# DataCanvasIO/DeepTables

Measured on AMD Instinct MI355X. Metric: training rows/sec (fwd+bwd) DeepFM Criteo-shape batch 8192, higher is better.
Workload: dtype f32 (split-bf16: 24-bit fwd / 16-bit bwd)

## Files before the change

### deeptables_amd/csrc/deepfm.hip

```cpp
#include <stdlib.h>
#include "tile_common.h"
#include "tower_x3.h"
#include "adam_dev.h"

namespace dt {

typedef float floatx4_t __attribute__((ext_vector_type(4)));

struct DeepFmAccum {
    int64_t dW1, dW2, db1, db2, dw3, dwo, dbo, loss, dgamma, dbeta, dwlin, slin, total;
    int64_t dw3d, dcw, dcb, sumc, sumcx;
};
__host__ __device__ inline DeepFmAccum deepfm_accum_layout(int C, int CP, int F, int Nd, int L = 0) {
    DeepFmAccum a;
    int64_t o = 0;
    a.dW1 = o; o += (int64_t)C * kH1;
    a.dW2 = o; o += (int64_t)kH1 * kH2;
    a.db1 = o; o += kH1;
    a.db2 = o; o += kH2;
    a.dw3 = o; o += (L > 0 ? C : 0);
    a.dw3d = o; o += kH2;
    a.dwo = o; o += 1;
    a.dbo = o; o += 1;
    a.loss = o; o += 2;
// ... 1528 lines not shown
                    acc[t][u] = __builtin_amdgcn_mfma_f32_32x32x16_bf16(al[t], bh[u], acc[t][u], 0, 0, 0);
                }
                acc[t][u] = __builtin_amdgcn_mfma_f32_32x32x16_bf16(ah[t], bh[u], acc[t][u], 0, 0, 0);
            }
    }
    auto put = [&](float* slot) {
#pragma unroll
        for (int t = 0; t < 2; ++t)
#pragma unroll
            for (int r = 0; r < 16; ++r) {
                const int i = (r & 3) + 8 * (r >> 2) + 4 * s;
                st4(slot + (2 * i + t) * 128 + 4 * c, floatx4{acc[t][0][r], acc[t][1][r], acc[t][2][r], acc[t][3][r]});
            }
    };
    put(red + wave * 8192);
    if (soft_cnt) {
        asm volatile("s_waitcnt lgkmcnt(0)" ::: "memory");
        if (lane == 0) atomicAdd(soft_cnt, 1u);
        while (*reinterpret_cast<volatile unsigned*>(soft_cnt) < 4u) __builtin_amdgcn_s_sleep(1);
        asm volatile("" ::: "memory");
    } else {
        __syncthreads();
    }
    float* dst = wpart + ((int64_t)mac * row_blocks + rb) * 8192;
#pragma unroll
    for (int u = 0; u < 8; ++u) {
        const int e = 4 * (tid + 256 * u);
        st4(dst + e, (ld4(red + e) + ld4(red + 8192 + e)) + (ld4(red + 16384 + e) + ld4(red + 24576 + e)));
    }
}

struct GPart {
    const float* part;
    int stride, tiles;
    float* gsum;
};
__device__ __forceinline__ void reduce_gpart(const GPart& gp, float* lds, int blk, int nblk, int tid, ElectSync& sy) {
    const int ee = tid & 15, tg = tid >> 4;
    for (int e0 = 16 * blk; e0 < gp.stride; e0 += 16 * nblk) {
        float acc = 0.f;
        for (int t0 = tg; t0 < gp.tiles; t0 += 16 * 8) {
            float v[8];
#pragma unroll
            for (int u = 0; u < 8; ++u) {
                const int t = t0 + 16 * u;
                const float x = gp.part[(int64_t)min(t, gp.tiles - 1) * gp.stride + e0 + ee];
                v[u] = t < gp.tiles ? x : 0.f;
            }
            acc += ((v[0] + v[1]) + (v[2] + v[3])) + ((v[4] + v[5]) + (v[6] + v[7]));
        }
        elect_barrier<256, true>(sy);
        lds[tg * 16 + ee] = acc;
        elect_barrier<256, true>(sy);
        if (tid < 16) {
            float t = 0.f;
#pragma unroll
            for (int g = 0; g < 16; ++g) t += lds[g * 16 + tid];
            gp.gsum[e0 + tid] = t;
        }
    }
}
struct X3Lay {
    __bf16 *W1B, *W1R, *W2B, *W2R;
    int64_t w1b_lo, w1r_lo, w2b_lo, w2r_lo;
    float* cwp;
};
__device__ __forceinline__ void x3_parts(float v, __bf16 (&q)[3]) {
    float r = v;
#pragma unroll
    for (int k = 0; k < 3; ++k) {
        const __bf16 a = (__bf16)r;
        q[k] = a;
        r -= (float)a;
    }
}

__device__ __forceinline__ void bn_grads2_body(const float* __restrict__ W1, const float* __restrict__ gamma,
                                               const float* __restrict__ beta, const DeepFmDims& dm, float* accum,
                                               const DeepFmAccum& al, const float* __restrict__ wpart, int row_blocks,
                                               int Lc, const float* __restrict__ cw, const float* __restrict__ cb,
                                               const float* __restrict__ w3c, const RecSrc& rs, const Part3& pl,
                                               floatx2 (*sm)[64], float* slin_s, const DenseAdam& da, int blk, const GPart& gp,
                                               const X3Lay& lay = X3Lay{nullptr, nullptr, nullptr, nullptr, 0, 0, 0, 0, nullptr}) {
    const int lane = threadIdx.x & 63, wave = threadIdx.x >> 6;
    if (blk == 0 && Lc == 0) {
        float* sl = reinterpret_cast<float*>(slin_s);
        for (int c = threadIdx.x; c < dm.C; c += blockDim.x) sl[c] = rec_sum(rs, pl.slin + c);
        __syncthreads();
        for (int q = threadIdx.x; q < dm.F + dm.Nd; q += blockDim.x) {
            float v = 0.f;
            if (q < dm.F) {
                for (int d = 0; d < dm.D; ++d) v += sl[q * dm.D + d];
            } else {
                v = sl[dm.F * dm.D + (q - dm.F)];
            }
            accum[al.dwlin + q] = v;
            if (da.p) adam_one(da.p, da.m, da.v, al.dwlin + q, v, da.lr_t, da.b1, da.b2, da.eps);
        }
    }
    const int col = blk;
    const bool w2 = col >= dm.C;
    const int mac = w2 ? (dm.CP >> 6) : (col >> 6), row = w2 ? col - dm.C : (col & 63);
    const float* src = wpart + (int64_t)mac * row_blocks * 8192 + row * 128 + 2 * lane;
    floatx2 w = {0.f, 0.f}, d = {0.f, 0.f};
    float ga = 0.f, be = 0.f;
    typedef double doublex2 __attribute__((ext_vector_type(2)));
    doublex2 dq[kRecShards];
#pragma unroll
    for (int sh = 0; sh < kRecShards; ++sh) dq[sh] = doublex2{0.0, 0.0};
    if (wave == 0 && !w2) {
        w = *reinterpret_cast<const floatx2*>(W1 + (int64_t)col * kH1 + 2 * lane);
#pragma unroll
        for (int sh = 0; sh < kRecShards; ++sh)
            dq[sh] = *reinterpret_cast<const doublex2*>(rs.racc + (int64_t)sh * rs.stride + pl.db1 + 2 * lane);
        ga = gamma[col]; be = beta[col];
    }
    const int64_t e0 = w2 ? al.dW2 + (int64_t)(2 * lane) * kH2 + row : al.dW1 + (int64_t)col * kH1 + 2 * lane;
    const int64_t e1 = w2 ? e0 + kH2 : e0 + 1;
    float pp[2] = {0.f, 0.f}, pm[2] = {0.f, 0.f}, pv[2] = {0.f, 0.f};
    if (da.p && wave == 0) {
        pp[0] = da.p[e0]; pp[1] = da.p[e1]; pm[0] = da.m[e0]; pm[1] = da.m[e1]; pv[0] = da.v[e0]; pv[1] = da.v[e1];
    }
    float pnew[2] = {0.f, 0.f};
    auto adam2 = [&](float g0, float g1) {
        const float g[2] = {g0, g1};
        const int64_t ei[2] = {e0, e1};
#pragma unroll
        for (int k = 0; k < 2; ++k) {
            const float mi = da.b1 * pm[k] + (1.f - da.b1) * g[k];
            const float vi = da.b2 * pv[k] + (1.f - da.b2) * g[k] * g[k];
            da.m[ei[k]] = mi;
            da.v[ei[k]] = vi;
            pnew[k] = pp[k] - da.lr_t * mi / (sqrtf(vi) + da.eps);
            da.p[ei[k]] = pnew[k];
        }
    };
    floatx2 v[8];
#pragma unroll
    for (int u = 0; u < 8; ++u) {
        const int sl = wave + 4 * u;
        v[u] = floatx2{0.f, 0.f};
        if (sl < row_blocks) v[u] = *reinterpret_cast<const floatx2*>(src + (int64_t)sl * 8192);
    }
    floatx2 m = ((v[0] + v[1]) + (v[2] + v[3])) + ((v[4] + v[5]) + (v[6] + v[7]));
    for (int sl = wave + 32; sl < row_blocks; sl += 4) m += *reinterpret_cast<const floatx2*>(src + (int64_t)sl * 8192);
    sm[wave][lane] = m;
    __syncthreads();
    if (wave != 0) return;
    m = (sm[0][lane] + sm[1][lane]) + (sm[2][lane] + sm[3][lane]);
    {
        doublex2 t = dq[0];
#pragma unroll
        for (int sh = 1; sh < kRecShards; ++sh) t += dq[sh];
        d = floatx2{(float)t[0], (float)t[1]};
    }
    if (w2) {
        accum[e0] = m.x;
        accum[e1] = m.y;
        if (da.p) adam2(m.x, m.y);
        if (da.p && lay.W1B) {
            __bf16 q0[3], q1[3];
            x3_parts(pnew[0], q0);
            x3_parts(pnew[1], q1);
            const int k0 = 2 * lane, n = row;
            const int64_t ib = ((((int64_t)(k0 >> 5) * 4 + (n >> 4)) * 64) + ((k0 >> 3) & 3) * 16 + (n & 15)) * 8 + (k0 & 7);
#pragma unroll
            for (int pt = 0; pt < 3; ++pt) {
// ... 20 lines not shown
            x3_parts(pnew[0], q0);
            x3_parts(pnew[1], q1);
            const int k = col, n0 = 2 * lane;
            const int64_t kb = ((int64_t)(k >> 5) * 8) * 64 * 8 + (((k >> 3) & 3) * 16) * 8 + (k & 7);
            const int64_t i0 = kb + ((int64_t)(n0 >> 4) * 64 + (n0 & 15)) * 8, i1 = kb + ((int64_t)((n0 + 1) >> 4) * 64 + ((n0 + 1) & 15)) * 8;
#pragma unroll
            for (int pt = 0; pt < 3; ++pt) {
                lay.W1B[pt * lay.w1b_lo + i0] = q0[pt];
                lay.W1B[pt * lay.w1b_lo + i1] = q1[pt];
            }
#pragma unroll
            for (int pt = 0; pt < 2; ++pt) {
                typedef __bf16 b2 __attribute__((ext_vector_type(2)));
                *reinterpret_cast<b2*>(lay.W1R + pt * lay.w1r_lo + (int64_t)k * kH1 + n0) = b2{q0[pt], q1[pt]};
            }
        }
    }
    if (Lc) {
        const int scal = pl.cross + (Lc + 1) * dm.CP;
        const int l = lane;
        const float sa_mine = l < Lc ? rec_sum(rs, scal + 16 + l) : 0.f;
        const float sco_mine = l <= Lc ? rec_sum(rs, scal + l) : 0.f;
        const float G = l <= Lc ? gp.gsum[(int64_t)l * dm.CP + col] : 0.f;
        const float sdz = rec_sum(rs, scal + 31);
        float cl = 0.f, suf = 0.f;
        for (int j = 0; j < Lc; ++j) {
            const float saj = __shfl(sa_mine, j, 64);
            const float bj = cb[(int64_t)j * dm.C + col], wj = cw[(int64_t)j * dm.C + col];
            if (j < l) cl += bj;
            if (j > l) suf += saj * wj;
        }
        if (l <= Lc) {
            const int64_t ig = l < Lc ? al.dcw + (int64_t)l * dm.C + col : al.dw3 + col;
            const float gw = ga_b * G + be_b * sco_mine + (l < Lc ? sa_mine : sdz) * cl;
            const float gb = sdz * w3c[col] + suf;
            accum[ig] = gw;
            if (l < Lc) accum[al.dcb + (int64_t)l * dm.C + col] = gb;
            if (da.p) {
                adam_one(da.p, da.m, da.v, ig, gw, da.lr_t, da.b1, da.b2, da.eps);
                if (l < Lc) adam_one(da.p, da.m, da.v, al.dcb + (int64_t)l * dm.C + col, gb, da.lr_t, da.b1, da.b2, da.eps);
                if (lay.cwp) {
                    lay.cwp[(int64_t)(l < Lc ? l : 2 * Lc) * dm.CP + col] = da.p[ig];
                    if (l < Lc) lay.cwp[(int64_t)(Lc + l) * dm.CP + col] = da.p[al.dcb + (int64_t)l * dm.C + col];
                }
            }
        }
    }
}

__global__ __launch_bounds__(256) void k_bn_grads2(const float* __restrict__ W1, const float* __restrict__ gamma,
                                                   const float* __restrict__ beta, DeepFmDims dm, float* accum,
                                                   DeepFmAccum al, const float* __restrict__ wpart, int row_blocks,
                                                   int Lc, const float* __restrict__ cw, const float* __restrict__ cb,
                                                   const float* __restrict__ w3c, RecSrc rs, int col_blocks, GPart gp) {
    __shared__ floatx2 sm[4][64];
    __shared__ float slin_s[kMaxC];
    const DenseAdam none{nullptr, nullptr, nullptr, 0.f, 0.f, 0.f, 0.f};
    const Part3 pl = part3_layout(dm.CP, Lc, 1);
    if ((int)blockIdx.x < col_blocks)
        bn_grads2_body(W1, gamma, beta, dm, accum, al, wpart, row_blocks, Lc, cw, cb, w3c, rs, pl, sm, slin_s, none, (int)blockIdx.x, gp);
    else
        finish_record_entry(((int)blockIdx.x - col_blocks) * (int)blockDim.x + (int)threadIdx.x, rs, pl, al, dm, Lc, accum, none);
}

__global__ __launch_bounds__(256) void k_finish_records(DeepFmDims dm, float* accum, DeepFmAccum al, int Lc, RecSrc rs,
                                                        double* __restrict__ bnacc_zero, int bnacc_n) {
    const DenseAdam none{nullptr, nullptr, nullptr, 0.f, 0.f, 0.f, 0.f};
    const Part3 pl = part3_layout(dm.CP, Lc, 0);
    const int i = (int)blockIdx.x * (int)blockDim.x + (int)threadIdx.x;
    finish_record_entry(i, rs, pl, al, dm, Lc, accum, none);
    for (int j = i; j < bnacc_n; j += (int)(gridDim.x * blockDim.x)) bnacc_zero[j] = 0.0;
}

struct FinishSeg {
    SegTail seg;
    float *table, *m, *v;
    const float* values;
    int sstride, D;
};
__global__ __launch_bounds__(256) void k_finish_step(const float* __restrict__ W1, const float* __restrict__ gamma,
                                                     const float* __restrict__ beta, DeepFmDims dm, float* accum,
                                                     DeepFmAccum al, const float* __restrict__ wpart, int row_blocks,
                                                     DenseAdam da, AdamState* __restrict__ st, float lr, int col_blocks,
                                                     int small_blocks, int seg_blocks, FinishSeg fs, int Lc,
                                                     const float* __restrict__ cw, const float* __restrict__ cb,
                                                     const float* __restrict__ w3c, RecSrc rs, X3Lay lay, GPart gp,
                                                     const float* __restrict__ lr_snap) {
    __shared__ floatx2 sm[4][64];
    __shared__ float slin_s[kMaxC];
    const Part3 pl = part3_layout(dm.CP, Lc, 1);
    const int sb = (int)blockIdx.x < seg_blocks ? (int)blockIdx.x : -1;
    const int b = sb >= 0 ? col_blocks + small_blocks : (int)blockIdx.x - seg_blocks < small_blocks
                      ? col_blocks + ((int)blockIdx.x - seg_blocks) : (int)blockIdx.x - seg_blocks - small_blocks;
    int nseg0 = 0;
    if (sb >= 0 && fs.seg.nseg) nseg0 = fs.seg.nseg[(sb * (int)(blockDim.x >> 6) + (int)(threadIdx.x >> 6)) % fs.seg.regions];
    if (lr_snap) da.lr_t = *lr_snap; else if (st) da.lr_t = st->lr_t;
    if (b < col_blocks) {
        bn_grads2_body(W1, gamma, beta, dm, accum, al, wpart, row_blocks, Lc, cw, cb, w3c, rs, pl, sm, slin_s, da, b, gp, lay);
    } else if (b < col_blocks + small_blocks) {
        finish_record_entry((b - col_blocks) * (int)blockDim.x + (int)threadIdx.x, rs, pl, al, dm, Lc, accum, da);
    } else if (fs.seg.nseg) {
        adam_segments<true>(fs.seg, seg_blocks, nseg0, fs.table, fs.m, fs.v, fs.values, fs.D, da.lr_t, da.b1, da.b2, da.eps,
                      fs.sstride, sb);
    }
    if (lr_snap) {
        if (blockIdx.x == 0 && threadIdx.x == 0 && st) {
            const int t = st->t + 1;
            st->t = t;
            st->lr_t = adam_lr_t(lr, da.b1, da.b2, t);
        }
    } else {
        __syncthreads();
        adam_finish(st, threadIdx.x == 0 ? 0u : kNoTicket, lr, da.b1, da.b2);
    }
}

__global__ void k_emb_drop_advance(unsigned* seed) { *seed = *seed * 1664525u + 1013904223u; }

struct RowsAdam {
    float *table, *m, *v;
    int sstride;
    const float* lr_t_dev;
    float lr_t_host, b1, b2, eps;
    int wt;
};
struct RowsEpi {
    const float *dXn, *X, *dz, *S, *wlin, *sc, *mean, *rstd;
    RecSrc rs;
    int sdx, sdxx;
    const int64_t* rows_out;
    float* grad_rows;
    float grad_scale;
    int field_major;
};
constexpr int kRowsUB = 4;

template <bool DCN>
__device__ __forceinline__ void rows_epilogue_wave(unsigned* work, int first_tile, int tile_stride, const DeepFmDims& dm,
                                                   const RowsEpi& a, const RowsAdam& ad, const EmbDrop& drop) {
    const int lane = threadIdx.x & 63, wv = threadIdx.x >> 6;
    const int LPR = dm.D >> 2, TPR = dm.F * LPR;
    const int parts = TPR > 64 ? 2 : 1;
    const int lpp = (TPR + parts - 1) / parts;
    const int rpw = parts == 1 ? 64 / TPR : 1;
    const int part = wv & (parts - 1);
    const int rsub = lane / lpp, pl = lane - rsub * lpp;
    const int piece = min(part * lpp + pl, TPR - 1);
    const bool active = rsub < rpw && part * lpp + pl < TPR;
    const int f = piece / LPR, c = piece - f * LPR;
    const int col = 4 * piece;
    const int tiles = (dm.B + kTM - 1) / kTM;
    const int chunk_rows = rpw * kRowsUB, chunks = (kTM + chunk_rows - 1) / chunk_rows;
    int dshift = 0;
    while ((1 << dshift) < dm.D) ++dshift;
    const floatx4 ca = ld4(a.sc + col), cmu = ld4(a.mean + col);
    floatx4 c1, c2;
    {
        typedef double doublex2 __attribute__((ext_vector_type(2)));
        doublex2 s1[2] = {{0.0, 0.0}, {0.0, 0.0}}, s2[2] = {{0.0, 0.0}, {0.0, 0.0}};
#pragma unroll
        for (int sh = 0; sh < kRecShards; ++sh) {
            const double* q = a.rs.racc + (int64_t)sh * a.rs.stride;
            s1[0] += *reinterpret_cast<const doublex2*>(q + a.sdx + col);
            s1[1] += *reinterpret_cast<const doublex2*>(q + a.sdx + col + 2);
            s2[0] += *reinterpret_cast<const doublex2*>(q + a.sdxx + col);
            s2[1] += *reinterpret_cast<const doublex2*>(q + a.sdxx + col + 2);
        }
        const floatx4 rsd = ld4(a.rstd + col);
        const float invN = 1.0f / (float)dm.B;
        c1 = floatx4{(float)s1[0][0], (float)s1[0][1], (float)s1[1][0], (float)s1[1][1]} * invN;
        c2 = rsd * floatx4{(float)s2[0][0], (float)s2[0][1], (float)s2[1][0], (float)s2[1][1]} * invN;
    }
    const float wl = DCN ? 0.f : a.wlin[f];
    const float lr_t = ad.lr_t_dev ? *ad.lr_t_dev : ad.lr_t_host;
    const unsigned dseed = drop.thr ? *drop.seed : 0u;
    for (;;) {
        unsigned it = 0;
        if (lane == 0) it = atomicAdd(&work[part], 1u);
        it = __builtin_amdgcn_readfirstlane(it);
        const int ti = (int)(it / (unsigned)chunks), ch = (int)(it - (unsigned)ti * (unsigned)chunks);
        const int tile = first_tile + ti * tile_stride;
        if (tile >= tiles) break;
        const int b0 = tile * kTM;
        {
            int64_t row[kRowsUB];
            floatx4 gx[kRowsUB], xr[kRowsUB], sv[kRowsUB];
            float dzv[kRowsUB];
            bool ok[kRowsUB];
            int bb[kRowsUB];
#pragma unroll
            for (int k = 0; k < kRowsUB; ++k) {
                const int r = ch * chunk_rows + k * rpw + rsub;
                ok[k] = active && r < kTM && b0 + r < dm.B;
                bb[k] = min(b0 + min(r, kTM - 1), dm.B - 1);
                row[k] = a.rows_out[(int64_t)bb[k] * dm.F + f];
            }
// ... 247 lines not shown
struct StepDense {
    float *p, *m, *v;
    int64_t n_flat;
    void* state;
    float lr;
};

struct StepChain {
    const void* next_idx;
    int64_t* next_rows_out;
    void* next_dedupe_ws;
};
static bool step_chains(const DeepFmDims& dm, int phases, bool with_dense, bool with_dedupe) {
    const bool x3_flag = (phases & (DT_STEP_TOWER_X3 | DT_STEP_TOWER_BF16)) != 0;
    return (phases & 0xf) == 2 && !(phases & (DT_STEP_SKIP_FINISH | DT_STEP_FINISH_ONLY)) && x3_flag && dm.CP <= 512 &&
           x3_fits(dm.CP) && with_dense && with_dedupe && dm.B <= kElectSlots && (int64_t)dm.B * dm.F < (1LL << 23);
}

extern "C" int dt_deepfm_step_chains(int B, int F, int D, int Nd, int phases) {
    DeepFmDims dm; int lpr;
    if (!deepfm_dims(B, F, D, Nd, &dm, &lpr)) return 0;
    return step_chains(dm, phases, true, true) ? 1 : 0;
}

namespace {
constexpr int kTraceEvents = 5, kTraceSteps = 32;
thread_local bool g_trace_on = false;
thread_local int g_trace_step = -1;
thread_local int g_trace_have[kTraceSteps];
thread_local hipEvent_t g_trace_ev[kTraceSteps][kTraceEvents];
thread_local bool g_trace_init = false;
inline void trace_mark(int i, hipStream_t st) {
    if (!g_trace_on) return;
    if (!g_trace_init) {
        for (int s = 0; s < kTraceSteps; ++s) {
            g_trace_have[s] = 0;
            for (int e = 0; e < kTraceEvents; ++e) g_trace_ev[s][e] = nullptr;
        }
        g_trace_init = true;
    }
    if (i == 0) { ++g_trace_step; g_trace_have[g_trace_step % kTraceSteps] = 0; }
    if (g_trace_step < 0) return;
    const int s = g_trace_step % kTraceSteps;
    if (g_trace_have[s] != i) return;
    if (!g_trace_ev[s][i]) hipEventCreate(&g_trace_ev[s][i]);
    hipEventRecord(g_trace_ev[s][i], st);
    g_trace_have[s] = i + 1;
}
}

extern "C" int dt_step_trace(int enable) {
    g_trace_on = enable != 0;
    g_trace_step = -1;
    if (g_trace_init) for (int s = 0; s < kTraceSteps; ++s) g_trace_have[s] = 0;
    return DT_OK;
}

extern "C" int dt_step_trace_read(float* us_host, int n, int* steps_host) {
    DT_REQUIRE(us_host && n >= kTraceEvents - 1, "dt_step_trace_read: us_host must take %d floats", kTraceEvents - 1);
    double sum[kTraceEvents - 1] = {0, 0, 0, 0};
    int steps = 0;
    if (g_trace_init && g_trace_step >= 0) {
        const int last = g_trace_step % kTraceSteps;
        if (g_trace_have[last] == kTraceEvents && hipEventSynchronize(g_trace_ev[last][kTraceEvents - 1]) != hipSuccess) {
            dt::set_error("dt_step_trace_read: hipEventSynchronize failed");
            return DT_ERR_LAUNCH;
        }
        for (int s = 0; s < kTraceSteps; ++s) {
            if (g_trace_have[s] != kTraceEvents) continue;
            bool ok = true;
            float ms[kTraceEvents - 1];
            for (int i = 0; i + 1 < kTraceEvents && ok; ++i)
                ok = hipEventElapsedTime(&ms[i], g_trace_ev[s][i], g_trace_ev[s][i + 1]) == hipSuccess;
            if (!ok) continue;
            for (int i = 0; i + 1 < kTraceEvents; ++i) sum[i] += ms[i] * 1e3;
            ++steps;
        }
    }
    DT_REQUIRE(steps > 0, "dt_step_trace_read: no traced step with the in-step optimizer on this thread "
               "(dt_step_trace(1), then dt_deepfm_train_step_adam / dt_dcn_train_step_adam)");
    for (int i = 0; i + 1 < kTraceEvents; ++i) us_host[i] = (float)(sum[i] / steps);
    if (steps_host) *steps_host = steps;
    return DT_OK;
}

static int tower_train_step(
    const void* idx, int idx_kind, const float* table, const int64_t* row_offset, const int32_t* vocab,
    const float* dense, const float* y, int B, int F, int D, int Nd,
    const float* w_lin, const float* bn_gamma, const float* bn_beta, float* bn_moving_mean,
    float* bn_moving_var, float bn_eps, float bn_momentum, const float* W1, const float* b1, const float* W2,
    const float* b2, const float* w3, const float* w_out, const float* b_out,
    float* logit_out, int64_t* rows_out, float* grad_rows, float* accum, void* workspace, int* oob_count,
    void* dedupe_ws, int64_t dedupe_slots, float grad_rows_scale, int grad_rows_field_major, int phases,
    float embedding_dropout, unsigned* dropout_seed, float dense_input_dropout,
    const float* sample_weight, void* stream, const float* cross_w, const float* cross_b, int Lc,
    const RowsAdam* adam = nullptr, const StepDense* sdense = nullptr, const StepChain* chain = nullptr) {
    DeepFmDims dm; int lpr;
    DT_UNSUPPORTED(!deepfm_dims(B, F, D, Nd, &dm, &lpr), "dt_deepfm_train_step: unsupported shape B=%d F=%d D=%d Nd=%d",
                   B, F, D, Nd);
    const bool dcn = Lc > 0;
    DT_REQUIRE(idx && table && row_offset && vocab && y && (dcn || w_lin) && bn_gamma && bn_beta && W1 && b1 && W2 && b2 &&
                   w3 && w_out && logit_out && rows_out && grad_rows && accum && workspace,
               "dt_deepfm_train_step: null pointer");
    DT_REQUIRE(Nd == 0 || dense, "dt_deepfm_train_step: dense is null");
    DT_REQUIRE(idx_kind == DT_IDX_F32 || idx_kind == DT_IDX_I32, "dt_deepfm_train_step: idx_kind %d", idx_kind);
    hipStream_t st = as_stream(stream);
    const DeepFmWs wl = deepfm_ws_layout(dm, Lc);
    const DeepFmAccum al = deepfm_accum_layout(dm.C, dm.CP, F, Nd, Lc);
    float* ws = reinterpret_cast<float*>(workspace);
    const int mse = (phases & DT_STEP_LOSS_MSE) ? 1 : 0;
    const bool skip_finish = (phases & DT_STEP_SKIP_FINISH) != 0, finish_only = (phases & DT_STEP_FINISH_ONLY) != 0;
    const bool bf16_flag = (phases & DT_STEP_TOWER_BF16) != 0;
    const bool x3_flag = (phases & DT_STEP_TOWER_X3) != 0 || bf16_flag;
    const bool prepared = (phases & DT_STEP_PREPARED) != 0;
    const bool preelected = (phases & DT_STEP_PREELECTED) != 0 || prepared;
    const int phases_all = phases;
    const bool stamps_flag = (phases & DT_STEP_STAMPS) != 0;
    phases &= 0xf;
    DT_REQUIRE(!(skip_finish && finish_only), "dt_deepfm_train_step: DT_STEP_SKIP_FINISH and DT_STEP_FINISH_ONLY together");
    const DcnArgs dca{cross_w, cross_b, w3, Lc, ws + wl.dXc, mse, 0, sample_weight, ws + wl.gpart, (Lc + 1) * dm.CP};
    const GPart gpt{dcn ? ws + wl.gpart : nullptr, (Lc + 1) * dm.CP, ceil_div(B, kTM), ws + wl.gsum};
    MlpParams mp{b1, W2, b2, dcn ? w3 + dm.C : w3, w_out, b_out, bn_gamma, ws + wl.mean, ws + wl.rstd, ws + wl.sc, ws + wl.betap,
                 W1, ws + wl.W1L, ws + wl.W2L, ws + wl.W2TL,
                 reinterpret_cast<const double*>(ws + wl.bnacc), bn_beta, bn_eps, bn_momentum, bn_moving_mean, bn_moving_var,
                 ws + wl.mean, ws + wl.rstd, ws + wl.sc, ws + wl.betap, ws + wl.gammap};
    DT_REQUIRE(((uintptr_t)W1 | (uintptr_t)W2 | (uintptr_t)(dcn ? W2 : w3) | (uintptr_t)accum) % 16 == 0,
               "dt_deepfm_train_step: W1 / W2 / w3 / accum must be 16-byte aligned");
    const int tiles = ceil_div(B, kTM);
    DedupeWs dd{nullptr, 0, nullptr, nullptr, nullptr, nullptr, nullptr};
    DT_REQUIRE(!(dedupe_ws && grad_rows_field_major), "dt_deepfm_train_step: dedupe and field-major row gradients "
                                                      "are mutually exclusive");
    if (dedupe_ws && phases >= 2) {
        DT_REQUIRE(dedupe_slots == (int64_t)B * F, "dt_deepfm_train_step: dedupe_slots=%lld must be "
                   "dt_deepfm_dedupe_slots(B, F)", (long long)dedupe_slots);
        DT_UNSUPPORTED((int64_t)B * F >= (1LL << 23), "dt_deepfm_train_step: the in-step dedupe takes up to 2^23 lookups (B=%d, F=%d)",
                       B, F);
        DT_REQUIRE((uintptr_t)dedupe_ws % 16 == 0, "dt_deepfm_train_step: dedupe_ws must be 16-byte aligned");
        dd = dedupe_view(dedupe_ws, dedupe_layout(B, F));
    }
    DT_REQUIRE(!preelected || (dd.rows_fm && !grad_rows_field_major),
               "dt_deepfm_train_step: DT_STEP_PREELECTED needs a backward step with dedupe_ws (filled by dt_deepfm_preelect)");
    if (B % kTM) {
        const int64_t pad = (int64_t)tiles * kTM - B;
        hipMemsetAsync(ws + wl.X + (int64_t)B * dm.CP, 0, (size_t)pad * dm.CP * sizeof(float), st);
        hipMemsetAsync(ws + wl.dH1 + (int64_t)B * kH1, 0, (size_t)pad * kH1 * sizeof(float), st);
    }
    EmbDrop drop{0u, 1.f, dropout_seed, 0u, 1.f};
    if (dense_input_dropout > 0.f && Nd > 0) {
        DT_REQUIRE(dense_input_dropout < 1.f && dropout_seed, "dt_deepfm_train_step: dense_input_dropout %f needs a rate < 1 "
                                                               "and the device seed word", dense_input_dropout);
        const double t = (double)dense_input_dropout * 4294967296.0;
        drop.thr_dense = t >= 4294967295.0 ? 4294967295u : (unsigned)t;
        if (drop.thr_dense == 0) drop.thr_dense = 1;
        drop.inv_keep_dense = 1.0f / (1.0f - dense_input_dropout);
    }
    if (embedding_dropout > 0.f) {
        DT_REQUIRE(embedding_dropout < 1.f && dropout_seed, "dt_deepfm_train_step: embedding_dropout %f needs a rate < 1 and "
                                                             "the device seed word", embedding_dropout);
        const double t = (double)embedding_dropout * 4294967296.0;
        drop.thr = t >= 4294967295.0 ? 4294967295u : (unsigned)t;
        if (drop.thr == 0) drop.thr = 1;
        drop.inv_keep = 1.0f / (1.0f - embedding_dropout);
    }
    unsigned long long* stamps = stamps_flag ? reinterpret_cast<unsigned long long*>(ws + wl.stamps) : nullptr;
    const bool pipe = phases >= 2;
    DT_REQUIRE(!(skip_finish || finish_only) || (pipe && !adam),
// ... 70 lines not shown
    PrepOut po{ws + wl.W1L, ws + wl.W2L,
               ws + wl.W2TL, W2, x3 ? x3_w1b : nullptr, x3_w1r, x3_w2b, x3_w2r, n1, n1, n2, n2,
               x3 && dcn ? x3_cwp : nullptr, cross_w, cross_b, w3, Lc};
    const int elect_blocks = (dd.rows_fm && !preelected) ? ((((F + 7) >> 3) << 3) << dd.parts_log2) : 0;
    const size_t ldsB = elect_blocks ? (dd.seg_cur ? kElectLdsBig : kElectLds) : 0;
    if (ldsB) hipFuncSetAttribute((const void*)k_prep, hipFuncAttributeMaxDynamicSharedMemorySize, (int)ldsB);
    if (!prepared) hipLaunchKernelGGL(k_prep, dim3(56 + elect_blocks), dim3(1024), ldsB, st, dm, W1, po, 56, dd, rows_out);
    trace_mark(1, st);
    {
#define DT_C(N)                                                                                                     \
    case N:                                                                                                         \
        if (dcn && pipe) {                                                                                          \
            hipFuncSetAttribute((const void*)k_mlp_fwd3<N, kCrossMax, true>, hipFuncAttributeMaxDynamicSharedMemorySize, (int)ldsC); \
            hipLaunchKernelGGL((k_mlp_fwd3<N, kCrossMax, true>), dim3(tiles), dim3(256), ldsC, st, ws + wl.X, mp, dm, \
                               ws + wl.lin, ws + wl.fm, y, ws + wl.H1, ws + wl.dH1, ws + wl.dH2, ws + wl.z,         \
                               logit_out, ws + wl.dlogit, ws + wl.dz, racc, stamps, dca, ws + wl.dXn);      \
        } else if (dcn) {                                                                                           \
            hipFuncSetAttribute((const void*)k_mlp_fwd3<N, kCrossMax>, hipFuncAttributeMaxDynamicSharedMemorySize, (int)ldsC); \
            hipLaunchKernelGGL((k_mlp_fwd3<N, kCrossMax>), dim3(tiles), dim3(256), ldsC, st, ws + wl.X, mp, dm,     \
                               ws + wl.lin, ws + wl.fm, y, ws + wl.H1, ws + wl.dH1, ws + wl.dH2, ws + wl.z,         \
                               logit_out, ws + wl.dlogit, ws + wl.dz, racc, stamps, dca, nullptr);          \
        } else if (pipe) {                                                                                          \
            hipFuncSetAttribute((const void*)k_mlp_fwd3<N, 0, true>, hipFuncAttributeMaxDynamicSharedMemorySize, (int)ldsC); \
            hipLaunchKernelGGL((k_mlp_fwd3<N, 0, true>), dim3(tiles), dim3(256), ldsC, st, ws + wl.X, mp, dm, ws + wl.lin, \
                               ws + wl.fm, y, ws + wl.H1, ws + wl.dH1, ws + wl.dH2, ws + wl.z, logit_out,           \
                               ws + wl.dlogit, ws + wl.dz, racc, stamps, dca, ws + wl.dXn);                 \
        } else {                                                                                                    \
            hipFuncSetAttribute((const void*)k_mlp_fwd3<N, 0>, hipFuncAttributeMaxDynamicSharedMemorySize, (int)ldsC); \
            hipLaunchKernelGGL((k_mlp_fwd3<N, 0>), dim3(tiles), dim3(256), ldsC, st, ws + wl.X, mp, dm, ws + wl.lin, \
                               ws + wl.fm, y, ws + wl.H1, ws + wl.dH1, ws + wl.dH2, ws + wl.z, logit_out,           \
                               ws + wl.dlogit, ws + wl.dz, racc, stamps, dca, nullptr);                     \
        }                                                                                                           \
        break;
#define DT_CXL(N, LCV, ONEV)                                                                                        \
    do {                                                                                                            \
        hipFuncSetAttribute((const void*)k_tower_x3<N, LCV, ONEV>, hipFuncAttributeMaxDynamicSharedMemorySize, (int)ldsX); \
        hipLaunchKernelGGL((k_tower_x3<N, LCV, ONEV>), dim3(tiles), dim3(512), ldsX, st, ws + wl.X, mp, xw, dm,     \
                           ws + wl.lin, ws + wl.fm, y, ws + wl.H1, ws + wl.dH1, ws + wl.dH2, ws + wl.z,             \
                           logit_out, ws + wl.dlogit, ws + wl.dz, racc, stamps, dca, ws + wl.dXn);          \
    } while (0)
#define DT_CX(N)                                                                                                    \
    case N: {                                                                                                       \
        const size_t ldsX = x3_lds_bytes(64 * N, dcn);                                                              \
        if (dcn) { if (bf16_flag) DT_CXL(N, kCrossMax, true); else DT_CXL(N, kCrossMax, false); }                   \
        else { if (bf16_flag) DT_CXL(N, 0, true); else DT_CXL(N, 0, false); }                                       \
    } break;
        if (x3) {
            switch (dm.CP >> 6) { DT_CX(1) DT_CX(2) DT_CX(3) DT_CX(4) DT_CX(5) DT_CX(6) DT_CX(7) DT_CX(8) }
        } else {
            switch (dm.CP >> 6) { DT_C(1) DT_C(2) DT_C(3) DT_C(4) DT_C(5) DT_C(6) DT_C(7) DT_C(8) DT_C(9) }
        }
#undef DT_CX
#undef DT_CXL
#undef DT_C
    }
    trace_mark(2, st);
    const Part3 pl3 = part3_layout(dm.CP, Lc, pipe ? 1 : 0);
    const RecSrc rsrc{racc, pl3.stride};
    const int rec_blocks = ceil_div(pl3.n, 256);
    if (pipe) {
        const int nmac = (dm.CP >> 6) + 1;
        const int row_blocks = wgrad_row_blocks();
        const int rows_per_block = ((B + row_blocks - 1) / row_blocks + 7) & ~7;
        const size_t ldsE = (size_t)4 * 8192 * sizeof(float);
        const RowsEpi ep{ws + wl.dXn, ws + wl.X, ws + wl.dz, ws + wl.S, w_lin, ws + wl.sc, ws + wl.mean, ws + wl.rstd,
                         rsrc, pl3.sdx, pl3.sdxx, rows_out, grad_rows, grad_rows_scale, grad_rows_field_major};
        RowsAdam ad = adam ? *adam : RowsAdam{nullptr, nullptr, nullptr, 0, nullptr, 0.f, 0.f, 0.f, 0.f, 0};
        const int join_env = 1;
        const int wm = (!x3 || stamps) ? 0 : bf16_flag ? 1 : 2;
#define DT_ED(DCNV, WMV)                                                                                                  \
    do {                                                                                                                  \
        hipFuncSetAttribute((const void*)k_wgrad_rows<DCNV, WMV>, hipFuncAttributeMaxDynamicSharedMemorySize, (int)ldsE);   \
        hipLaunchKernelGGL((k_wgrad_rows<DCNV, WMV>), dim3(nmac * row_blocks), dim3(512), ldsE, st, ws + wl.X, mp, dm,       \
                           ws + wl.H1, ws + wl.dH1, ws + wl.dH2, row_blocks, rows_per_block, ws + wl.wpart,                \
                           stamps ? stamps + (int64_t)tiles * 32 : nullptr, ep, ad, drop,                                 \
                           stamps ? stamps + (int64_t)tiles * 16 : nullptr, join_env, bnacc, (int)wl.bnacc_n, nx, gpt,    \
                           (adam && sdense) ? ws + wl.lrsnap : nullptr);                                               \
    } while (0)
        if (dcn) { if (wm == 0) DT_ED(true, 0); else if (wm == 1) DT_ED(true, 1); else DT_ED(true, 2); }
        else { if (wm == 0) DT_ED(false, 0); else if (wm == 1) DT_ED(false, 1); else DT_ED(false, 2); }
#undef DT_ED
        trace_mark(3, st);
        if (adam && sdense) {
            const int seg_blocks = 1024;
            const int small_blocks = rec_blocks;
            const DedupeLayout dl = dedupe_layout(B, F);
            const FinishSeg fs{SegTail{dd.nseg, dd.seg_row, dd.seg_off, dd.seg_cnt, dd.seg_list, dl.regions, dl.cap},
                               adam->table, adam->m, adam->v, grad_rows, adam->sstride, D};
            const DenseAdam da{sdense->p, sdense->m, sdense->v, adam->lr_t_host, adam->b1, adam->b2, adam->eps};
            const X3Lay lay = nx.idx ? X3Lay{x3_w1b, x3_w1r, x3_w2b, x3_w2r, n1, n1, n2, n2, dcn ? x3_cwp : nullptr}
                                     : X3Lay{nullptr, nullptr, nullptr, nullptr, 0, 0, 0, 0, nullptr};
            hipLaunchKernelGGL(k_finish_step, dim3(dm.C + kH2 + small_blocks + seg_blocks), dim3(256), 0, st, W1, ws + wl.gammap,
                               ws + wl.betap, dm, accum, al, ws + wl.wpart, row_blocks, da, (AdamState*)sdense->state, sdense->lr,
                               dm.C + kH2, small_blocks, seg_blocks, fs, Lc, cross_w, cross_b, w3, rsrc, lay, gpt, ws + wl.lrsnap);
            trace_mark(4, st);
        } else if (!skip_finish) {
            hipLaunchKernelGGL(k_bn_grads2, dim3(dm.C + kH2 + rec_blocks), dim3(256), 0, st, W1, bn_gamma, bn_beta, dm,
                               accum, al, ws + wl.wpart, row_blocks, Lc, cross_w, cross_b, w3, rsrc, dm.C + kH2, gpt);
        }
        if ((drop.thr || drop.thr_dense) && !skip_finish)
            hipLaunchKernelGGL(k_emb_drop_advance, dim3(1), dim3(1), 0, st, dropout_seed);
    } else {
        hipLaunchKernelGGL(k_finish_records, dim3(max(rec_blocks, 8)), dim3(256), 0, st, dm, accum, al, Lc, rsrc, bnacc,
                           (int)wl.bnacc_n);
    }
    return launch_status(dcn ? "dt_dcn_train_step" : "dt_deepfm_train_step");
}

extern "C" int dt_deepfm_train_step(
    const void* idx, int idx_kind, const float* table, const int64_t* row_offset, const int32_t* vocab,
    const float* dense, const float* y, int B, int F, int D, int Nd,
    const float* w_lin, const float* bn_gamma, const float* bn_beta, float* bn_moving_mean,
    float* bn_moving_var, float bn_eps, float bn_momentum, const float* W1, const float* b1, const float* W2,
    const float* b2, const float* w3, const float* w_out, const float* b_out,
    float* logit_out, int64_t* rows_out, float* grad_rows, float* accum, void* workspace, int* oob_count,
    void* dedupe_ws, int64_t dedupe_slots, float grad_rows_scale, int grad_rows_field_major, int phases,
    float embedding_dropout, unsigned* dropout_seed, float dense_input_dropout,
    const float* sample_weight, void* stream) {
    DT_REQUIRE(w_lin, "dt_deepfm_train_step: null pointer");
    return tower_train_step(idx, idx_kind, table, row_offset, vocab, dense, y, B, F, D, Nd, w_lin, bn_gamma, bn_beta,
                            bn_moving_mean, bn_moving_var, bn_eps, bn_momentum, W1, b1, W2, b2, w3, w_out, b_out, logit_out,
                            rows_out, grad_rows, accum, workspace, oob_count, dedupe_ws, dedupe_slots, grad_rows_scale,
                            grad_rows_field_major, phases, embedding_dropout, dropout_seed, dense_input_dropout, sample_weight, stream, nullptr, nullptr, 0);
}

struct StepAdam {
    RowsAdam ad;
    StepDense sd;
    StepChain ch;
};
static int step_adam_args(const char* what, float* table, int D, void* dedupe_ws, int phases, float* adam_m, float* adam_v,
                          int slot_stride, void* adam_state, float lr_t, float beta1, float beta2, float eps, float* dense_p,
                          float* dense_m, float* dense_v, int64_t dense_n, float lr, const void* next_idx,
                          int64_t* next_rows_out, void* next_dedupe_ws, StepAdam* out) {
    DT_REQUIRE(table && adam_m && adam_v, "%s: null pointer", what);
    DT_REQUIRE(dense_n == 0 || (dense_p && dense_m && dense_v && adam_state),
               "%s: the dense half needs the flat buffers and the device step state", what);
    DT_REQUIRE((phases & 0xf) == 2 && dedupe_ws, "%s: a backward step (phases 2) with dedupe_ws", what);
    DT_REQUIRE(slot_stride == D || slot_stride == 2 * D, "%s: slot_stride %d (D or 2 D)", what, slot_stride);
    DT_REQUIRE(((uintptr_t)table | (uintptr_t)adam_m | (uintptr_t)adam_v) % 16 == 0,
               "%s: table / slots must be 16-byte aligned", what);
    out->ad = RowsAdam{table, adam_m, adam_v, slot_stride, adam_state ? adam_state_lr_t(adam_state) : nullptr, lr_t, beta1,
                       beta2, eps, 0};
    out->sd = StepDense{dense_p, dense_m, dense_v, dense_n, adam_state, lr};
    out->ch = StepChain{next_idx, next_rows_out, next_dedupe_ws};
    return DT_OK;
}

extern "C" int dt_deepfm_train_step_adam(
    const void* idx, int idx_kind, float* table, const int64_t* row_offset, const int32_t* vocab,
    const float* dense, const float* y, int B, int F, int D, int Nd,
    const float* w_lin, const float* bn_gamma, const float* bn_beta, float* bn_moving_mean,
    float* bn_moving_var, float bn_eps, float bn_momentum, const float* W1, const float* b1, const float* W2,
    const float* b2, const float* w3, const float* w_out, const float* b_out,
    float* logit_out, int64_t* rows_out, float* grad_rows, float* accum, void* workspace, int* oob_count,
    void* dedupe_ws, int64_t dedupe_slots, int phases, float embedding_dropout, unsigned* dropout_seed, float dense_input_dropout,
    const float* sample_weight,
    float* adam_m, float* adam_v, int slot_stride, void* adam_state, float lr_t, float beta1, float beta2,
    float eps, float* dense_p, float* dense_m, float* dense_v, int64_t dense_n, float lr,
    const void* next_idx, int64_t* next_rows_out, void* next_dedupe_ws, void* stream) {
    DT_REQUIRE(w_lin, "dt_deepfm_train_step_adam: null pointer");
    StepAdam a;
    const int rc = step_adam_args("dt_deepfm_train_step_adam", table, D, dedupe_ws, phases, adam_m, adam_v, slot_stride,
                                  adam_state, lr_t, beta1, beta2, eps, dense_p, dense_m, dense_v, dense_n, lr, next_idx,
                                  next_rows_out, next_dedupe_ws, &a);
    if (rc != DT_OK) return rc;
    return tower_train_step(idx, idx_kind, table, row_offset, vocab, dense, y, B, F, D, Nd, w_lin, bn_gamma, bn_beta,
                            bn_moving_mean, bn_moving_var, bn_eps, bn_momentum, W1, b1, W2, b2, w3, w_out, b_out, logit_out,
                            rows_out, grad_rows, accum, workspace, oob_count, dedupe_ws, dedupe_slots, 1.0f, 0, phases,
                            embedding_dropout, dropout_seed, dense_input_dropout, sample_weight, stream, nullptr, nullptr, 0, &a.ad,
                            dense_n > 0 ? &a.sd : nullptr, &a.ch);
}

extern "C" int dt_dcn_supported(int B, int F, int D, int Nd, int H1, int H2, int L) {
    DeepFmDims dm; int lpr;
    if (!dt_deepfm_supported(B, F, D, Nd, H1, H2) || L < 1 || L > kCrossMax) return 0;
    if (!deepfm_dims(B, F, D, Nd, &dm, &lpr)) return 0;
// ... 76 lines not shown
```

Baseline: 82.80 million.

## Make finish-step kernel persistent with grid-stride loops over all work types

The finish kernel used to launch one block per column, per record chunk and per segment slice (over a thousand segment blocks). It now launches a fixed grid of two blocks per CU, and every block runs the segment Adam, the record-entry finish and a strided loop over the BN/weight-grad columns in turn. This cuts block scheduling overhead and tail effects, and it removes the adam_finish ticket path by always using lr_snap. The costs are serialisation of heterogeneous work inside each block and extra __syncthreads between columns. The code now assumes lr_snap is non-null, and a volatile asm stops the compiler from folding threadIdx arithmetic.

```diff
diff --git a/deeptables_amd/csrc/deepfm.hip b/deeptables_amd/csrc/deepfm.hip
--- a/deeptables_amd/csrc/deepfm.hip
+++ b/deeptables_amd/csrc/deepfm.hip
@@ -1634,7 +1634,9 @@
                                                const float* __restrict__ w3c, const RecSrc& rs, const Part3& pl,
                                                floatx2 (*sm)[64], float* slin_s, const DenseAdam& da, int blk, const GPart& gp,
                                                const X3Lay& lay = X3Lay{nullptr, nullptr, nullptr, nullptr, 0, 0, 0, 0, nullptr}) {
-    const int lane = threadIdx.x & 63, wave = threadIdx.x >> 6;
+    int tid = (int)threadIdx.x;
+    asm volatile("" : "+v"(tid));
+    const int lane = tid & 63, wave = tid >> 6;
     if (blk == 0 && Lc == 0) {
         float* sl = reinterpret_cast<float*>(slin_s);
         for (int c = threadIdx.x; c < dm.C; c += blockDim.x) sl[c] = rec_sum(rs, pl.slin + c);
@@ -1821,36 +1823,30 @@
                                                      const float* __restrict__ beta, DeepFmDims dm, float* accum,
                                                      DeepFmAccum al, const float* __restrict__ wpart, int row_blocks,
                                                      DenseAdam da, AdamState* __restrict__ st, float lr, int col_blocks,
-                                                     int small_blocks, int seg_blocks, FinishSeg fs, int Lc,
+                                                     FinishSeg fs, int Lc,
                                                      const float* __restrict__ cw, const float* __restrict__ cb,
                                                      const float* __restrict__ w3c, RecSrc rs, X3Lay lay, GPart gp,
                                                      const float* __restrict__ lr_snap) {
     __shared__ floatx2 sm[4][64];
     __shared__ float slin_s[kMaxC];
     const Part3 pl = part3_layout(dm.CP, Lc, 1);
-    const int sb = (int)blockIdx.x < seg_blocks ? (int)blockIdx.x : -1;
-    const int b = sb >= 0 ? col_blocks + small_blocks : (int)blockIdx.x - seg_blocks < small_blocks
-                      ? col_blocks + ((int)blockIdx.x - seg_blocks) : (int)blockIdx.x - seg_blocks - small_blocks;
+    const int blk = (int)blockIdx.x, grid = (int)gridDim.x;
     int nseg0 = 0;
-    if (sb >= 0 && fs.seg.nseg) nseg0 = fs.seg.nseg[(sb * (int)(blockDim.x >> 6) + (int)(threadIdx.x >> 6)) % fs.seg.regions];
-    if (lr_snap) da.lr_t = *lr_snap; else if (st) da.lr_t = st->lr_t;
-    if (b < col_blocks) {
+    if (fs.seg.nseg) nseg0 = fs.seg.nseg[(blk * (int)(blockDim.x >> 6) + (int)(threadIdx.x >> 6)) % fs.seg.regions];
+    da.lr_t = *lr_snap;
+    if (fs.seg.nseg)
+        adam_segments<true>(fs.seg, grid, nseg0, fs.table, fs.m, fs.v, fs.values, fs.D, da.lr_t, da.b1, da.b2, da.eps,
+                            fs.sstride, blk);
+    for (int e = blk * (int)blockDim.x + (int)threadIdx.x; e < pl.n; e += grid * (int)blockDim.x)
+        finish_record_entry(e, rs, pl, al, dm, Lc, accum, da);
+    for (int b = blk; b < col_blocks; b += grid) {
+        if (b != blk) __syncthreads();
         bn_grads2_body(W1, gamma, beta, dm, accum, al, wpart, row_blocks, Lc, cw, cb, w3c, rs, pl, sm, slin_s, da, b, gp, lay);
-    } else if (b < col_blocks + small_blocks) {
-        finish_record_entry((b - col_blocks) * (int)blockDim.x + (int)threadIdx.x, rs, pl, al, dm, Lc, accum, da);
-    } else if (fs.seg.nseg) {
-        adam_segments<true>(fs.seg, seg_blocks, nseg0, fs.table, fs.m, fs.v, fs.values, fs.D, da.lr_t, da.b1, da.b2, da.eps,
-                      fs.sstride, sb);
-    }
-    if (lr_snap) {
-        if (blockIdx.x == 0 && threadIdx.x == 0 && st) {
-            const int t = st->t + 1;
-            st->t = t;
-            st->lr_t = adam_lr_t(lr, da.b1, da.b2, t);
-        }
-    } else {
-        __syncthreads();
-        adam_finish(st, threadIdx.x == 0 ? 0u : kNoTicket, lr, da.b1, da.b2);
+    }
+    if (blk == 0 && threadIdx.x == 0 && st) {
+        const int t = st->t + 1;
+        st->t = t;
+        st->lr_t = adam_lr_t(lr, da.b1, da.b2, t);
     }
 }
 
@@ -2264,6 +2260,22 @@
     for (int i = 0; i + 1 < kTraceEvents; ++i) us_host[i] = (float)(sum[i] / steps);
     if (steps_host) *steps_host = steps;
     return DT_OK;
+}
+
+constexpr int kFinishBlocksPerCu = 2;
+static int finish_grid() {
+    static const int grid = [] {
+        if (const char* e = getenv("DT_AMD_FINISH_GRID")) {
+            const int g = atoi(e);
+            if (g > 0) return g < 65536 ? g : 65536;
+        }
+        int dev = 0, cus = 0;
+        if (hipGetDevice(&dev) != hipSuccess ||
+            hipDeviceGetAttribute(&cus, hipDeviceAttributeMultiprocessorCount, dev) != hipSuccess || cus <= 0)
+            cus = 256;
+        return kFinishBlocksPerCu * cus;
+    }();
+    return grid;
 }
 
 static int tower_train_step(
@@ -2500,17 +2512,15 @@
 #undef DT_ED
         trace_mark(3, st);
         if (adam && sdense) {
-            const int seg_blocks = 1024;
-            const int small_blocks = rec_blocks;
             const DedupeLayout dl = dedupe_layout(B, F);
             const FinishSeg fs{SegTail{dd.nseg, dd.seg_row, dd.seg_off, dd.seg_cnt, dd.seg_list, dl.regions, dl.cap},
                                adam->table, adam->m, adam->v, grad_rows, adam->sstride, D};
             const DenseAdam da{sdense->p, sdense->m, sdense->v, adam->lr_t_host, adam->b1, adam->b2, adam->eps};
             const X3Lay lay = nx.idx ? X3Lay{x3_w1b, x3_w1r, x3_w2b, x3_w2r, n1, n1, n2, n2, dcn ? x3_cwp : nullptr}
                                      : X3Lay{nullptr, nullptr, nullptr, nullptr, 0, 0, 0, 0, nullptr};
-            hipLaunchKernelGGL(k_finish_step, dim3(dm.C + kH2 + small_blocks + seg_blocks), dim3(256), 0, st, W1, ws + wl.gammap,
+            hipLaunchKernelGGL(k_finish_step, dim3(finish_grid()), dim3(256), 0, st, W1, ws + wl.gammap,
                                ws + wl.betap, dm, accum, al, ws + wl.wpart, row_blocks, da, (AdamState*)sdense->state, sdense->lr,
-                               dm.C + kH2, small_blocks, seg_blocks, fs, Lc, cross_w, cross_b, w3, rsrc, lay, gpt, ws + wl.lrsnap);
+                               dm.C + kH2, fs, Lc, cross_w, cross_b, w3, rsrc, lay, gpt, ws + wl.lrsnap);
             trace_mark(4, st);
         } else if (!skip_finish) {
             hipLaunchKernelGGL(k_bn_grads2, dim3(dm.C + kH2 + rec_blocks), dim3(256), 0, st, W1, bn_gamma, bn_beta, dm,
```

After: 80.76 million. -2.5%, worse.
